# open-forest-observatory/geograypher

Measured on AMD Instinct MI355X. Metric: Mpix/s rasterized (face-ID pix2face), 1.2M-face mesh @ 4000x3000, higher is better.
Workload: dtype int32 (fixed-point edge functions) / fp32 (vertex transform, depth); 1 GPU; BASELINE config 2: 1201250-face heightfield (V=602176), 50 pinhole views/GPU @ 4000x3000, f=3000 px, 120 m AGL lawn-mower grid, face-ID raster to int32 in HBM; faces=1201250, vertices=602176, parallelism=views sharded, mesh replicated, dp1

## Files before the change

geograypher_amd/csrc/binning.hip:

```cpp
#include "gr_internal.hpp"
#include "dev_common.hpp"

using namespace grimpl;

namespace {

struct Vtx {
  int X, Y;
  float iz;
  bool valid;
  bool front, finite;
};

__device__ __forceinline__ bool snap_vertex(float qx, float qy, float iz, const float *__restrict__ cam, int gl_order, int h, int w,
                                            int &X, int &Y) {
  if (!gl_order) {
    const float fx = cam[12] * qx;
    const float fy = cam[12] * qy;
    const float sx = cam[13] + fx * iz;
    const float sy = cam[14] + fy * iz;
    X = (int)floorf(sx * 256.0f + 0.5f);
    Y = (int)floorf(sy * 256.0f + 0.5f);
    return (fabsf(sx) < 16384.0f) && (fabsf(sy) < 16384.0f);
  }
// ... 1 lines not shown
  const float px = two_f / (float)w, py = -(two_f / (float)h);
  const float hw = 0.5f * (float)w, hh = 0.5f * (float)h;
  const float xc = px * qx, yc = py * qy;
  const float xn = xc * iz, yn = yc * iz;
  const float xw = __builtin_fmaf(xn, hw, hw), yw = __builtin_fmaf(yn, hh, hh);
  const float fx = (xw - 0.5f) * 256.0f, fy = (yw - 0.5f) * 256.0f;
  X = (int)rintf(fx) + 128;
  Y = 256 * h - 128 - (int)rintf(fy);
  return (fabsf(xw) < 16384.0f) && (fabsf(yw) < 16384.0f);
}

__device__ __forceinline__ Vtx project_vertex(const float *__restrict__ p, const float *__restrict__ cam, int gl_order, int h, int w) {
  Vtx v;
  const float dx = p[0] - cam[9];
  const float dy = p[1] - cam[10];
  const float dz = p[2] - cam[11];
  float m0, m1, m2;
  m0 = cam[0] * dx; m1 = cam[3] * dy; m2 = cam[6] * dz;
  const float qx = (m0 + m1) + m2;
  m0 = cam[1] * dx; m1 = cam[4] * dy; m2 = cam[7] * dz;
  const float qy = (m0 + m1) + m2;
  m0 = cam[2] * dx; m1 = cam[5] * dy; m2 = cam[8] * dz;
  const float qz = (m0 + m1) + m2;
  v.valid = qz > cam[15];
  v.front = v.valid;
  v.finite = isfinite(qx) && isfinite(qy) && isfinite(qz);
  const float iz = 1.0f / qz;
  const bool inside = snap_vertex(qx, qy, iz, cam, gl_order, h, w, v.X, v.Y);
  v.valid = v.valid && inside;
  v.iz = iz;
  return v;
}

__device__ __forceinline__ void wave_group(int t, int lane, int &leader, int &rank, int &size) {
  leader = lane; rank = 0; size = 0;
  unsigned long long rem = __ballot(t >= 0);
  while (rem) {
    const int l = __ffsll((long long)rem) - 1;
    const int tl = __builtin_amdgcn_readlane(t, l);
    const unsigned long long m = __ballot(t == tl);
    if (t == tl) {
      leader = l;
      rank = __popcll(m & ((1ull << lane) - 1ull));
      size = __popcll(m);
    }
    rem &= ~m;
  }
}

__device__ __forceinline__ void wave_group_weighted(int t, int w, int lane, int &leader, int &rank, int &size) {
  leader = lane; rank = 0; size = 0;
  unsigned long long rem = __ballot(t >= 0);
  const unsigned long long b0 = __ballot(((w - 1) & 1) != 0), b1 = __ballot(((w - 1) & 2) != 0);
  const unsigned long long low = (1ull << lane) - 1ull;
  while (rem) {
    const int l = __ffsll((long long)rem) - 1;
    const int tl = __builtin_amdgcn_readlane(t, l);
    const unsigned long long m = __ballot(t == tl);
    if (t == tl) {
      leader = l;
      rank = __popcll(m & low) + __popcll(m & low & b0) + 2 * __popcll(m & low & b1);
      size = __popcll(m) + __popcll(m & b0) + 2 * __popcll(m & b1);
    }
    rem &= ~m;
  }
}

__device__ __forceinline__ void wave_group_capped(int t, int lane, int &leader, int &rank, int &size, int max_groups) {
  leader = lane; rank = 0; size = 1;
  unsigned long long rem = __ballot(t >= 0);
  for (int g = 0; rem && g < max_groups; ++g) {
    const int l = __ffsll((long long)rem) - 1;
    const int tl = __builtin_amdgcn_readlane(t, l);
    const unsigned long long m = __ballot(t == tl);
    if (t == tl) {
      leader = l;
      rank = __popcll(m & ((1ull << lane) - 1ull));
      size = __popcll(m);
    }
    rem &= ~m;
  }
}

__global__ __launch_bounds__(256) void k_cull_blocks(const float *__restrict__ cams, BinArgs a, int nblk) {
  const int slot = blockIdx.y;
  const int b = blockIdx.x * 256 + threadIdx.x;
  const float *cam = cams + (int64_t)slot * GR_CAM_FLOATS;
  uint32_t *ctrl = a.ctrl + slot * a.ctrl_stride;
  bool keep = false;
  if (b < nblk) {
    const float4 sp = a.blk[b];
    const float dx = sp.x - cam[9], dy = sp.y - cam[10], dz = sp.z - cam[11];
    const float qx = cam[0] * dx + cam[3] * dy + cam[6] * dz;
    const float qy = cam[1] * dx + cam[4] * dy + cam[7] * dz;
    const float qz = cam[2] * dx + cam[5] * dy + cam[8] * dz;
    const float fe = fabsf(cam[12]), r = sp.w * 1.001f;
    const float mxl = cam[13] + 2.0f, mxr = (float)a.w - cam[13] + 2.0f;
    const float myt = cam[14] + 2.0f, myb = (float)a.h - cam[14] + 2.0f;
    bool out = (qz + r < cam[15]);
    out = out || (cam[12] * qx + mxl * qz < -r * (fe + fabsf(mxl)));
    out = out || (-cam[12] * qx + mxr * qz < -r * (fe + fabsf(mxr)));
    out = out || (cam[12] * qy + myt * qz < -r * (fe + fabsf(myt)));
    out = out || (-cam[12] * qy + myb * qz < -r * (fe + fabsf(myb)));
    keep = !out;
  }
  const unsigned long long m = __ballot(keep);
  if (m != 0ull) {
    const int lane = threadIdx.x & 63;
    const int leader = __ffsll((long long)m) - 1;
    uint32_t base = 0;
    if (lane == leader) base = atomicAdd(&ctrl[3], (uint32_t)__popcll(m));
    base = __shfl(base, leader);
    if (keep) a.work[(int64_t)slot * a.work_stride + base + __popcll(m & ((1ull << lane) - 1ull))] = (uint32_t)b;
  }
}

struct FaceForm {
  int Xf, Yf, dxf, dyf, tf, rf;
  int Xm, Ym, dxm, dym, tm, rm;
  int Xl, Yl, dxl, dyl, tl, rl;
  int X0, Y0;
  int w3, w4, w5;
  int ywf;
  bool fast;
  int jmin, jmax, imin, imax;
  int iz0, A, B, nface;
};

__device__ __forceinline__ FaceForm face_form(const int4 p0, const int4 p1, const int4 p2, int TW, int TH);
__device__ __forceinline__ bool tile_entry(const FaceForm &ff, int px0, int py0, int TW, int TH, int4 &e0, int4 &e1, int4 &e2,
                                           int &rows);
__device__ __forceinline__ bool compile_entry(const BinArgs &a, uint32_t *__restrict__ ctrl, int4 *__restrict__ comp,
                                              uint8_t *__restrict__ nr8, int64_t idx, const int4 p0, const int4 p1,
                                              const int4 p2, int px0, int py0, int TW, int TH);
__device__ __forceinline__ bool build_entry(const int4 p0, const int4 p1, const int4 p2, int px0, int py0, int TW, int TH,
                                            int4 &e0, int4 &e1, int4 &e2, int &rows);
__device__ __forceinline__ void store_entry(const BinArgs &a, uint32_t *__restrict__ ctrl, int4 *__restrict__ comp,
                                            uint8_t *__restrict__ nr8, int64_t idx, const int4 e0, const int4 e1, const int4 e2,
                                            int rows);
__device__ __forceinline__ void shifted_entry(const int4 b0, const int4 b1, const int4 b2, int boxx, int boxy, int px0, int py0, int dX,
                                              int dY, int TW, int TH, int4 &e0, int4 &e1, int4 &e2, int &rows);
#define GR_FAST_EXT 24000
__device__ __forceinline__ int pack16(int lo, int hi) { return (lo & 0xFFFF) | (hi << 16); }

__device__ __forceinline__ bool face_setup_tail(const BinArgs &a, int face_id, Vtx v0, Vtx v1, Vtx v2, int4 &r0, int4 &r1,
                                                int4 &r2, int &tx0, int &tx1, int &ty0, int &ty1, bool &clip_me) {
  clip_me = !(v0.valid && v1.valid && v2.valid) && (v0.front || v1.front || v2.front) && v0.finite && v1.finite && v2.finite;
  if (!(v0.valid && v1.valid && v2.valid)) return false;
  long long area2 = (long long)(v1.X - v0.X) * (long long)(v2.Y - v0.Y) - (long long)(v2.X - v0.X) * (long long)(v1.Y - v0.Y);
  if (area2 == 0) return false;
  if (area2 < 0) {
    Vtx s = v1; v1 = v2; v2 = s;
    area2 = -area2;
  }
  const int Xmin = imin3(v0.X, v1.X, v2.X), Xmax = imax3(v0.X, v1.X, v2.X);
  const int Ymin = imin3(v0.Y, v1.Y, v2.Y), Ymax = imax3(v0.Y, v1.Y, v2.Y);
  int jmin = (Xmin - 128 + 255) >> 8, jmax = (Xmax - 128) >> 8;
  int imin = (Ymin - 128 + 255) >> 8, imax = (Ymax - 128) >> 8;
  jmin = max(jmin, 0); imin = max(imin, 0);
  jmax = min(jmax, a.w - 1); imax = min(imax, a.h - 1);
  if (jmin > jmax || imin > imax) return false;
  const double d1 = (double)v1.iz - (double)v0.iz;
  const double d2 = (double)v2.iz - (double)v0.iz;
  const double a2 = (double)area2;
  double n1, n2;
  n1 = d1 * (double)(v2.Y - v0.Y); n2 = d2 * (double)(v1.Y - v0.Y);
  const float A = (float)((n1 - n2) / a2);
// ... 669 lines not shown
      const float dx = p[0] - cam[9], dy = p[1] - cam[10], dz = p[2] - cam[11];
      float m0, m1, m2;
      m0 = cam[0] * dx; m1 = cam[3] * dy; m2 = cam[6] * dz;
      px[0][k][tid] = (double)((m0 + m1) + m2);
      m0 = cam[1] * dx; m1 = cam[4] * dy; m2 = cam[7] * dz;
      py[0][k][tid] = (double)((m0 + m1) + m2);
      m0 = cam[2] * dx; m1 = cam[5] * dy; m2 = cam[8] * dz;
      pz[0][k][tid] = (double)((m0 + m1) + m2);
    }
    int n = 3, cur = 0;
    bool bad = false;
#pragma unroll
    for (int pl = 0; pl < 5; ++pl) {
      const double pa = pl == 1 ? -(double)fe : pl == 2 ? (double)fe : 0.0;
      const double pb = pl == 3 ? -(double)fe : pl == 4 ? (double)fe : 0.0;
      const double pc = pl == 0 ? 1.0 : pl == 1 ? G - (double)cxp : pl == 2 ? G + (double)cxp : pl == 3 ? G - (double)cyp
                                                                                                        : G + (double)cyp;
      const double pd = pl == 0 ? -(double)nearp : 0.0;
      const double plane[4] = {pa, pb, pc, pd};
      if (n == 0 || bad) break;
      int m = 0;
      for (int e = 0; e < n; ++e) {
        const int e1 = (e + 1) % n;
        const P3 S = {px[cur][e][tid], py[cur][e][tid], pz[cur][e][tid]};
        const P3 E = {px[cur][e1][tid], py[cur][e1][tid], pz[cur][e1][tid]};
        const double dS = clip_plane(plane, S), dE = clip_plane(plane, E);
        const bool inS = dS >= 0.0, inE = dE >= 0.0;
        P3 o0 = E, o1 = E;
        int cnt = 0;
        if (inS && inE) { cnt = 1; }
        else if (inS && !inE) { o0 = clip_cross(S, dS, E, dE); cnt = 1; }
        else if (!inS && inE) { o0 = clip_cross(E, dE, S, dS); cnt = 2; }
        if (cnt >= 1) { if (m < 8) { px[cur ^ 1][m][tid] = o0.x; py[cur ^ 1][m][tid] = o0.y; pz[cur ^ 1][m][tid] = o0.z; } ++m; }
        if (cnt == 2) { if (m < 8) { px[cur ^ 1][m][tid] = o1.x; py[cur ^ 1][m][tid] = o1.y; pz[cur ^ 1][m][tid] = o1.z; } ++m; }
      }
      if (m > 8) bad = true;
      n = m;
      cur ^= 1;
    }
    if (bad || n < 3) continue;
    for (int e = 0; e < n; ++e) {
      const float qx = (float)px[cur][e][tid], qy = (float)py[cur][e][tid], qz = (float)pz[cur][e][tid];
      if (!(qz > 0.0f)) { bad = true; break; }
      const float iz = 1.0f / qz;
      int Xs, Ys;
      if (!snap_vertex(qx, qy, iz, cam, a.gl_order, a.h, a.w, Xs, Ys)) { bad = true; break; }
      sX[e][tid] = Xs;
      sY[e][tid] = Ys;
      sZ[e][tid] = iz;
    }
    if (bad) continue;
    const int face = a.orig[f];
    Vtx v0;
    v0.X = sX[0][tid]; v0.Y = sY[0][tid]; v0.iz = sZ[0][tid]; v0.valid = v0.front = v0.finite = true;
    for (int k = 1; k + 1 < n; ++k) {
      Vtx v1 = v0, v2 = v0;
      v1.X = sX[k][tid]; v1.Y = sY[k][tid]; v1.iz = sZ[k][tid];
      v2.X = sX[k + 1][tid]; v2.Y = sY[k + 1][tid]; v2.iz = sZ[k + 1][tid];
      emit_triangle<DIRECT>(a, slot, ctrl, v0, v1, v2, face);
    }
  }
}

__global__ __launch_bounds__(256) void k_bin_init(uint4 *__restrict__ ctrl16, int64_t n16, uint32_t *__restrict__ touched, int64_t nt,
                                                  unsigned long long *__restrict__ stats) {
  const int64_t i0 = (int64_t)blockIdx.x * 256 + threadIdx.x, step = (int64_t)gridDim.x * 256;
  for (int64_t i = i0; i < n16; i += step) ctrl16[i] = make_uint4(0u, 0u, 0u, 0u);
  for (int64_t i = i0; i < nt; i += step) touched[i] = 0u;
  if (stats && i0 < 11) stats[i0] = i0 == 4 ? ~0ull : 0ull;
}

__global__ __launch_bounds__(256) void k_sum_visits(const uint32_t *__restrict__ visits, int64_t n, unsigned long long *__restrict__ out) {
  unsigned long long sum = 0;
  for (int64_t i = (int64_t)blockIdx.x * 256 + threadIdx.x; i < n; i += (int64_t)gridDim.x * 256) sum += visits[i];
  for (int o = 32; o > 0; o >>= 1) sum += __shfl_xor(sum, o);
  if ((threadIdx.x & 63) == 0 && sum) atomicAdd(out, sum);
}

}

namespace grimpl {

int bin_batch(gr_ctx *c, const float *cams, int nb, int h, int w, int slot0, int group, hipStream_t s) {
  BinArgs a = make_args(c, h, w, slot0);
  a.group = group;
  {
    const int64_t n16 = c->ctrl_stride * nb / 4;
    const int64_t nt = a.touched ? (int64_t)nb * a.tw : 0;
    const unsigned blocks = (unsigned)std::max<int64_t>(1, std::min<int64_t>(ceil_div(std::max(n16, nt), 256), 2048));
    unsigned long long *const st = c->stats_pending ? c->stats : nullptr;
    GR_LAUNCH_EV((hipEvent_t) nullptr, chain_begin(c), k_bin_init, dim3(blocks), dim3(256), 0, s, reinterpret_cast<uint4 *>(a.ctrl), n16, a.touched, nt, st);
    c->stats_pending = false;
  }
  if (a.dbg & 512) {
    GR_HIP(c, hipMemsetAsync(a.comp, 0xFF, sizeof(int4) * GR_ENT_Q * (size_t)c->ent_cap * nb, s));
    GR_HIP(c, hipMemsetAsync(a.nrow8, 0xFF, (size_t)c->ent_cap * nb, s));
  }
  {
    const int nblk = (int)ceil_div(c->F, GR_BLOCK);
    hipLaunchKernelGGL(k_cull_blocks, dim3((unsigned)ceil_div(nblk, 256), nb), dim3(256), 0, s,
                       cams, a, nblk);
    const int gmax = std::min((nblk + 3) / 4, 1024);
    const dim3 gsetup((unsigned)std::max(1, std::min(gmax, std::max(nblk / 128, 4096 / std::max(nb, 1)))), nb);
    if (a.cap_tile > 0) {
      if (a.micro) hipLaunchKernelGGL((k_setup_cull<true, true>), gsetup, dim3(256), 0, s, cams, a);
      else hipLaunchKernelGGL((k_setup_cull<true, false>), gsetup, dim3(256), 0, s, cams, a);
      GR_LAUNCH_EV((hipEvent_t) nullptr, chain_stop(c, ST_SETUP), k_clip_faces<true>, dim3(8, nb), dim3(64), 0, s, cams, a);
    } else {
      hipLaunchKernelGGL((k_setup_cull<false, false>), gsetup, dim3(256), 0, s, cams, a);
      GR_LAUNCH_EV((hipEvent_t) nullptr, chain_stop(c, ST_SETUP), k_clip_faces<false>, dim3(8, nb), dim3(64), 0, s, cams, a);
    }
  }
  c->last_direct = a.cap_tile > 0;
  if (a.cap_tile > 0) {
    if (c->defer_stats) {
      c->stats_deferred = true; c->deferred_args = a; c->deferred_nb = nb;
    } else {
      GR_LAUNCH_EV((hipEvent_t) nullptr, chain_stop(c, ST_SCAN), k_bin_stats, dim3(nb), dim3(1024), 0, s, a);
    }
  } else {
    GR_LAUNCH_EV((hipEvent_t) nullptr, chain_stop(c, ST_SCAN), k_scan_tiles, dim3(nb), dim3(1024), 0, s, a);
    {
      const unsigned g = (unsigned)std::min<int64_t>(ceil_div(c->F, 256), 1024);
      GR_LAUNCH_EV((hipEvent_t) nullptr, chain_stop(c, ST_FILL), k_fill_compile, dim3(g, nb), dim3(256), 0, s, a);
    }
  }
  GR_HIP(c, hipGetLastError());
  return GR_OK;
}

int sum_visits(gr_ctx *c, hipStream_t s) {
  if (!c->visits_pending) return GR_OK;
  c->visits_pending = false;
  hipLaunchKernelGGL(k_sum_visits, dim3(64), dim3(256), 0, s, c->visits, ceil_div(c->F, 64), c->stats + 7);
  GR_HIP(c, hipGetLastError());
  return GR_OK;
}

int bin_stats_deferred(gr_ctx *c, hipStream_t s) {
  if (!c->stats_deferred) return GR_OK;
  c->stats_deferred = false;
  hipLaunchKernelGGL(k_bin_stats, dim3(c->deferred_nb), dim3(1024), 0, s, c->deferred_args);
  GR_HIP(c, hipGetLastError());
  return GR_OK;
}

}
```

geograypher_amd/csrc/geograster.hip:

```cpp

#include <unistd.h>

#include <mutex>
#include <new>

#include "gr_internal.hpp"

using namespace grimpl;

namespace {

std::mutex g_learned_mu;
gr_ctx::Learned g_learned[64];
int g_n_learned = 0;
char g_learned_path[1024] = {0};

#define GR_LEARNED_EXACT (-1)
#define GR_LEARNED_MAX_CAP 65536

inline int merge_cap(int a, int b) { return (a == GR_LEARNED_EXACT || b == GR_LEARNED_EXACT) ? GR_LEARNED_EXACT : std::max(a, b); }

void put_global_locked(const gr_ctx::Learned &v);

bool parse_learned_line(const char *line, gr_ctx::Learned &v) {
// ... 27 lines not shown

void put_global_locked(const gr_ctx::Learned &v) {
  int j = 0;
  for (; j < std::min(g_n_learned, 64); ++j)
    if (g_learned[j].mesh == v.mesh && g_learned[j].T == v.T) break;
  if (j == std::min(g_n_learned, 64)) {
    j = g_n_learned % 64; g_n_learned += 1;
    g_learned[j] = v;
    return;
  }
  g_learned[j].cap = merge_cap(g_learned[j].cap, v.cap);
  g_learned[j].full = g_learned[j].full || v.full;
  g_learned[j].micro = g_learned[j].micro || v.micro;
}

void lookup_learned(const gr_ctx *c, int T, int &cap, bool &full, bool *micro = nullptr) {
  cap = 0; full = false;
  if (micro) *micro = false;
  for (int i = 0; i < std::min(c->n_learned, 8); ++i)
    if (c->learned[i].mesh == c->mesh_sig && c->learned[i].T == T) {
      cap = c->learned[i].cap; full = c->learned[i].full;
      if (micro) *micro = c->learned[i].micro;
      return;
    }
  if (c->share_learned) {
    std::lock_guard<std::mutex> lk(g_learned_mu);
    for (int i = 0; i < std::min(g_n_learned, 64); ++i)
      if (g_learned[i].mesh == c->mesh_sig && g_learned[i].T == T) {
        cap = g_learned[i].cap; full = g_learned[i].full;
        if (micro) *micro = g_learned[i].micro;
        return;
      }
  }
}

void resolve_binning(gr_ctx *c, int T) {
  int cap = 0; bool full = false, micro = false;
  c->cur_cap = 0; c->cur_ent40 = false; c->cur_micro = false; c->cur_look = false; c->cur_count_micro = false;
  if (c->opt_direct_cap <= 0 || !c->direct_ok) return;
  lookup_learned(c, T, cap, full, &micro);
  if (cap == GR_LEARNED_EXACT) return;
  c->cur_look = cap == 0 && !(c->opt_var & 16384);
  c->cur_cap = std::max(cap, c->opt_direct_cap);
  c->cur_ent40 = !(c->cur_cap & 63) && !(c->opt_var & 128) && !full;
  c->cur_micro = c->cur_ent40 && !(c->opt_var & 4096) && (micro || (c->opt_var & 8192));
  c->cur_count_micro = c->cur_ent40 && !c->cur_micro && !(c->opt_var & 4096) && (c->cur_look || (c->opt_var & 16384));
}

void learn(gr_ctx *c, int T, int cap, bool full, bool micro = false) {
  int old_cap; bool old_full, old_micro;
  lookup_learned(c, T, old_cap, old_full, &old_micro);
  const gr_ctx::Learned v = {c->mesh_sig, T, merge_cap(cap, old_cap), full || old_full, micro || old_micro};
  int i = 0;
  for (; i < std::min(c->n_learned, 8); ++i)
    if (c->learned[i].mesh == c->mesh_sig && c->learned[i].T == T) break;
  if (i == std::min(c->n_learned, 8)) { i = c->n_learned % 8; c->n_learned += 1; }
  c->learned[i] = v;
  if (!c->share_learned) return;
  std::lock_guard<std::mutex> lk(g_learned_mu);
  put_global_locked(v);
  save_learned_locked();
}

void learn_slots(gr_ctx *c, int T, int64_t max_tile, bool full, bool micro) {
  const int64_t need = (max_tile + max_tile / 8 + 16 + 63) / 64 * 64;
  const int64_t bytes_one_view = need * (16 * GR_ENT_Q) * (int64_t)T;
  if (need <= GR_LEARNED_MAX_CAP && bytes_one_view <= (c->opt_budget_mb << 20)) learn(c, T, (int)need, full, micro);
  else learn(c, T, GR_LEARNED_EXACT, full, micro);
}

int ensure_bins(gr_ctx *c, int n_slots, int T) {
  const int64_t F = c->F > 0 ? c->F : 1;
  const int dcap = c->cur_cap;
  const bool direct = dcap > 0;
  int64_t cap = c->ent_cap_request > 0 ? c->ent_cap_request : (F / 2 + 65536);
  if (direct) cap = std::max<int64_t>(cap, (int64_t)T * dcap);
  int clg = -1;
  if (direct && !(c->opt_var & 131072)) {
    if (T <= 1024) { clg = 0; while ((1 << clg) < T + 3) ++clg; }
  }
  const int Tcap = clg < 0 ? ((T + 3) & ~3) : (32 << clg);
  const int64_t ctrl_stride = ((GR_CTRL_HDR + (direct ? 2 : 4) * (int64_t)Tcap) + 63) / 64 * 64;
  const int64_t work_stride = ceil_div(F, GR_BLOCK) + 4;
  int rc = grow(c, c->ctrl, c->ctrl_have, ctrl_stride * n_slots, "bin control");
  if (!rc) rc = grow(c, c->comp, c->comp_have, GR_ENT_Q * cap * n_slots, "entry list");
  if (!rc) rc = grow(c, c->nrow8, c->nrow_have, cap * n_slots + 64, "entry row counts");
  if (!rc) rc = grow(c, c->work, c->work_have, work_stride * n_slots, "work list");
  if (!rc) rc = grow(c, c->clip, c->clip_have, F * n_slots, "clip list");
  const int64_t RF = std::max<int64_t>(F, c->rec_cap_request);
  if (!rc && !direct) rc = grow(c, c->rec, c->rec_have, 4 * RF * n_slots, "record planes");
  if (rc) return rc;
  c->slots = n_slots; c->Tcap = Tcap; c->clg = clg; c->ent_cap = cap; c->ctrl_stride = ctrl_stride; c->work_stride = work_stride;
  c->rec_F = RF; c->rec_stride = 4 * RF;
  return GR_OK;
}

int raster_views(gr_ctx *c, const float *cams, int n_views, int h, int w, int32_t *ids, float *depth,
                 const uint8_t *labels, int C, uint32_t *votes, uint32_t *counts, int flags, hipStream_t s, int again = 0) {
  int rc = check_common(c, n_views, h, w);
  if (rc) return rc;
  c->rebinned = again;
  if (again == 0) c->causes = 0;
  if (!c->verts) return fail(c, GR_ENOMESH, "gr_mesh_upload has not been called");
  if (!cams) return fail(c, GR_EINVAL, "null cams");
  if (n_views == 0) return GR_OK;
  GR_HIP(c, hipSetDevice(c->device));
  int B = n_views < c->opt_batch ? n_views : c->opt_batch;
  const int thl = c->opt_thl;
  const int T = ((w + GR_TILE - 1) >> GR_TILE_LOG2) * ((h + (1 << thl) - 1) >> thl);
  resolve_binning(c, T);
  {
    const int64_t per_slot = (int64_t)T * c->cur_cap * (16 * GR_ENT_Q);
    if (per_slot > 0) B = (int)std::max<int64_t>(1, std::min<int64_t>(B, (c->opt_budget_mb << 20) / per_slot));
  }
  rc = ensure_bins(c, B, T);
  if (rc) return rc;
  c->last_T = T; c->last_B = B;
  const int64_t P = (int64_t)h * w, F = c->F;
  const bool overlap = labels && n_views > B && !(c->opt_var & 4);
  const int tw = (int)ceil_div(ceil_div(F, 64), 4);
  const bool use_touched = labels != nullptr;
  if (labels) {
    rc = ensure_winner(c, sizeof(uint32_t) * (size_t)F * B * (overlap ? 2 : 1), s);
    if (rc) return rc;
    if (use_touched) {
      rc = grow(c, c->touched, c->touched_have, (int64_t)2 * B * tw, "winner group maps");
      if (!rc) rc = grow(c, c->visits, c->visits_have, ceil_div(F, 64) + 4, "visit counters");
      if (rc) return rc;
      if (again == 0) GR_HIP(c, hipMemsetAsync(c->visits, 0, sizeof(uint32_t) * (size_t)(ceil_div(F, 64) + 4), s));
      c->visits_pending = true;
    }
    if (overlap && !c->side) {
      GR_HIP(c, hipStreamCreateWithFlags(&c->side, hipStreamNonBlocking));
      for (int i = 0; i < 2; ++i) {
        GR_HIP(c, hipEventCreateWithFlags(&c->ev_raster[i], hipEventDisableTiming));
        GR_HIP(c, hipEventCreateWithFlags(&c->ev_vote[i], hipEventDisableTiming));
      }
    }
  }
  c->last_stream = s;
  note_stream(c, s);
  c->stats_pending = true;
  c->stats_deferred = false;
  if (!labels) c->visits_pending = false;
  c->defer_stats = !labels && n_views <= B && !(c->cur_look && again < 2);
  c->last_n_views = n_views;
  int g = 0;
  for (int v0 = 0; v0 < n_views; v0 += B, ++g) {
    const int nb = (n_views - v0) < B ? (n_views - v0) : B;
    const int buf = overlap ? (g & 1) : 0;
    uint32_t *tch = use_touched ? c->touched + (int64_t)buf * B * tw : nullptr;
    if (tch) {
      if (overlap && g >= 2) GR_HIP(c, hipStreamWaitEvent(s, c->ev_vote[buf], 0));
    }
    c->cur_touched = tch; c->cur_tw = tw;
    rc = bin_batch(c, cams + (int64_t)v0 * GR_CAM_FLOATS, nb, h, w, 0, v0 / B, s);
    c->cur_touched = nullptr;
    if (rc) return rc;
    if (c->cur_look && g == 0 && again < 2) {
      unsigned long long st[11] = {0, 0, 0, 0, 0, 0, 0, 0, 0, 0, 0};
      GR_HIP(c, hipMemcpyAsync(st, c->stats, sizeof(st), hipMemcpyDeviceToHost, s));
      GR_HIP(c, hipStreamSynchronize(s));
      c->causes |= (int)(st[10] & 7u);
      const bool grow = st[3] && (int64_t)st[2] > c->cur_cap, miss = st[3] && st[5] != 0;
      const bool micro = !c->cur_micro && !(c->opt_var & (128 | 4096)) && !miss && st[0] > 0 && 5 * st[8] > 2 * st[0];
      if (grow) learn_slots(c, T, (int64_t)st[2], miss, micro);
      else learn(c, T, c->cur_cap, miss, micro);
      if (grow || miss || micro) return raster_views(c, cams, n_views, h, w, ids, depth, labels, C, votes, counts, flags, s, again + 1);
    }
    uint32_t *win = labels ? (uint32_t *)c->winner + (int64_t)buf * F * B : nullptr;
    RasterOut out;
    out.ids = ids ? ids + v0 * P : nullptr;
    out.depth = depth ? depth + v0 * P : nullptr;
    out.winner = win;
    out.touched = reinterpret_cast<uint8_t *>(tch);
    out.tb = 4 * (int64_t)tw;
    out.F = F;
    out.compat = (flags & GR_FLAG_NEG1_IS_LAST_FACE) ? 1 : 0;
    if (overlap && g >= 2) GR_HIP(c, hipStreamWaitEvent(s, c->ev_vote[buf], 0));
    rc = tile_batch(c, nb, h, w, 0, out, s);
    if (rc) return rc;
    if (labels) {
      hipStream_t vs = s;
      if (overlap) {
        GR_HIP(c, hipEventRecord(c->ev_raster[buf], s));
        GR_HIP(c, hipStreamWaitEvent(c->side, c->ev_raster[buf], 0));
        vs = c->side;
      }
      launch_vote_labels(c, vs, win, labels + v0 * P, nb, F, P, C, votes, counts, v0 / B, (const uint32_t *)tch, tw, flags);
      GR_HIP(c, hipGetLastError());
      if (overlap) GR_HIP(c, hipEventRecord(c->ev_vote[buf], c->side));
    }
  }
  if (overlap) {
    GR_HIP(c, hipStreamWaitEvent(s, c->ev_vote[(g - 1) & 1], 0));
    if (g >= 2) GR_HIP(c, hipStreamWaitEvent(s, c->ev_vote[g & 1], 0));
  }
  return GR_OK;
}

}

extern "C" {

int gr_version(void) { return GR_VERSION; }

int gr_ctx_create(int device, gr_ctx **out) {
  if (!out) return GR_EINVAL;
  *out = nullptr;
  int n = 0;
  if (hipGetDeviceCount(&n) != hipSuccess || n <= 0 || device < 0 || device >= n) return GR_ENODEVICE;
  if (hipSetDevice(device) != hipSuccess) return GR_ENODEVICE;
  gr_ctx *c = new (std::nothrow) gr_ctx();
  if (!c) return GR_ENOMEM;
  c->device = device;
  if (hipMalloc(&c->stats, sizeof(unsigned long long) * 16) != hipSuccess ||
      hipMalloc(&c->flag, sizeof(int) * 8) != hipSuccess) {
    delete c;
    return GR_ENOMEM;
  }
  (void)hipMemset(c->stats, 0, sizeof(unsigned long long) * 16);
  (void)hipDeviceSynchronize();
#ifdef GR_STAMPS
  if (hipMalloc(&c->stamps, sizeof(unsigned long long) * 32 * 1024) == hipSuccess) (void)hipMemset(c->stamps, 0, sizeof(unsigned long long) * 32 * 1024);
#endif
  *out = c;
  return GR_OK;
}

int gr_ctx_destroy(gr_ctx *c) {
  if (!c) return GR_OK;
  (void)hipSetDevice(c->device);
  (void)hipDeviceSynchronize();
  for (auto &sp : c->spans) { if (sp.own_a) (void)hipEventDestroy(sp.a); (void)hipEventDestroy(sp.b); }
  for (auto e : c->pool) (void)hipEventDestroy(e);
  if (c->ctrl) (void)hipFree(c->ctrl);
  if (c->rec) (void)hipFree(c->rec);
  if (c->comp) (void)hipFree(c->comp);
  if (c->nrow8) (void)hipFree(c->nrow8);
  if (c->work) (void)hipFree(c->work);
  if (c->clip) (void)hipFree(c->clip);
  if (c->winner) (void)hipFree(c->winner);
  for (int i = 0; i < 2; ++i) {
    if (c->ev_raster[i]) (void)hipEventDestroy(c->ev_raster[i]);
    if (c->ev_vote[i]) (void)hipEventDestroy(c->ev_vote[i]);
  }
  if (c->side) (void)hipStreamDestroy(c->side);
  if (c->sort_tmp) (void)hipFree(c->sort_tmp);
  if (c->resize_tmp) (void)hipFree(c->resize_tmp);
  if (c->blk) (void)hipFree(c->blk);
// ... 38 lines not shown
    case GR_OPT_DIRECT_CAP:
      if (value < 0 || value > 65536) return fail(c, GR_EINVAL, "slots per tile must be in [0, 65536]");
      c->opt_direct_cap = value; c->direct_ok = true; c->n_learned = 0; c->share_learned = false; return GR_OK;
    case GR_OPT_SHARE_LEARNED:
      c->share_learned = value != 0; return GR_OK;
    case GR_OPT_VERTEX_ORDER:
      if (value != 0 && value != 1) return fail(c, GR_EINVAL, "vertex order must be 0 (rule R1) or 1 (OpenGL's order of operations)");
      c->opt_gl_order = value; return GR_OK;
    case GR_OPT_DIRECT_BUDGET_MB:
      if (value < 1) return fail(c, GR_EINVAL, "entry-memory budget must be at least 1 MiB");
      c->opt_budget_mb = value; return GR_OK;
    default: return fail(c, GR_EINVAL, "unknown option %d", key);
  }
}

int gr_learned_cache_file(const char *path_h) {
  std::lock_guard<std::mutex> lk(g_learned_mu);
  if (!path_h || !path_h[0]) { g_learned_path[0] = 0; return GR_OK; }
  if (strlen(path_h) >= sizeof(g_learned_path)) return GR_EINVAL;
  snprintf(g_learned_path, sizeof(g_learned_path), "%s", path_h);
  FILE *f = fopen(path_h, "r");
  if (!f) return GR_OK;
  char line[256];
  gr_ctx::Learned v;
  while (fgets(line, sizeof(line), f))
    if (parse_learned_line(line, v)) put_global_locked(v);
  fclose(f);
  return GR_OK;
}

int gr_learned_cache_clear(void) {
  std::lock_guard<std::mutex> lk(g_learned_mu);
  g_n_learned = 0;
  memset(g_learned, 0, sizeof(g_learned));
  return GR_OK;
}

#ifdef GR_STAMPS
int gr_debug_read_stamps(gr_ctx *c, unsigned long long *out16_h) {
  if (!c || !out16_h || !c->stamps) return GR_EINVAL;
  GR_HIP(c, hipDeviceSynchronize());
  std::vector<unsigned long long> all(16 * 1024);
  GR_HIP(c, hipMemcpy(all.data(), c->stamps, sizeof(unsigned long long) * all.size(), hipMemcpyDeviceToHost));
  GR_HIP(c, hipMemset(c->stamps, 0, sizeof(unsigned long long) * all.size()));
  for (int k = 0; k < 16; ++k) out16_h[k] = 0;
  for (size_t i = 0; i < all.size(); ++i) out16_h[i & 15] += all[i];
  return GR_OK;
}
#endif

#ifdef GR_STAMPS
int gr_debug_read_setup_stamps(gr_ctx *c, unsigned long long *out16_h) {
  if (!c || !out16_h || !c->stamps) return GR_EINVAL;
  GR_HIP(c, hipDeviceSynchronize());
  std::vector<unsigned long long> all(16 * 1024);
  GR_HIP(c, hipMemcpy(all.data(), c->stamps + 16 * 1024, sizeof(unsigned long long) * all.size(), hipMemcpyDeviceToHost));
  GR_HIP(c, hipMemset(c->stamps + 16 * 1024, 0, sizeof(unsigned long long) * all.size()));
  for (int k = 0; k < 16; ++k) out16_h[k] = 0;
  for (size_t i = 0; i < all.size(); ++i) out16_h[i & 15] += all[i];
  return GR_OK;
}
#endif

int gr_get_stage_times(gr_ctx *c, gr_stage_times *o) {
  if (!c || !o) return GR_EINVAL;
  float acc[ST_N] = {0};
  for (auto &sp : c->spans) {
    GR_HIP(c, hipEventSynchronize(sp.b));
    float ms = 0.f;
    GR_HIP(c, hipEventElapsedTime(&ms, sp.a, sp.b));
    acc[sp.stage] += ms;
  }
  o->setup_ms = acc[ST_SETUP]; o->scan_ms = acc[ST_SCAN]; o->fill_ms = acc[ST_FILL]; o->raster_ms = acc[ST_RASTER];
  o->project_ms = acc[ST_PROJECT]; o->vote_ms = acc[ST_VOTE]; o->gather_ms = acc[ST_GATHER];
  o->raster_launches = c->prof_raster_launches; o->views = c->prof_views;
  release_spans(c);
  c->prof_views = 0; c->prof_raster_launches = 0;
  return GR_OK;
}

int gr_raster_face_ids(gr_ctx *c, const float *cams, int n_views, int h, int w, int32_t *ids, float *depth,
                       void *stream) {
  if (c && !ids && !depth) return fail(c, GR_EINVAL, "null outputs");
  return raster_views(c, cams, n_views, h, w, ids, depth, nullptr, 0, nullptr, nullptr, 0, (hipStream_t)stream);
}

int gr_raster_status(gr_ctx *c, gr_raster_stats *o) {
  if (!c || !o) return GR_EINVAL;
  unsigned long long st[11] = {0, 0, 0, 0, 0, 0, 0, 0, 0, 0, 0};
  {
    int rc = bin_stats_deferred(c, c->last_stream);
    if (!rc) rc = sum_visits(c, c->last_stream);
    if (rc) return rc;
  }
  GR_HIP(c, hipMemcpyAsync(st, c->stats, sizeof(st), hipMemcpyDeviceToHost, c->last_stream));
  GR_HIP(c, hipStreamSynchronize(c->last_stream));
  o->records = (int64_t)st[0]; o->entries = (int64_t)st[1]; o->max_entries = (int64_t)st[2];
  o->entry_cap = c->ent_cap; o->overflow = (int32_t)st[3];
  o->blocks = (int64_t)st[6]; o->chunk_visits = (int64_t)st[7];
  o->rebinned_groups = c->rebinned;
  c->causes |= (int)(st[10] & 7u);
  o->views_done = st[3] ? (int32_t)std::min<unsigned long long>(st[4] * (unsigned long long)std::max(c->last_B, 1),
                                                                (unsigned long long)c->last_n_views)
                        : c->last_n_views;
  if (st[3] && c->last_direct) {
    const int used = c->cur_cap;
    const bool grow = (int64_t)st[2] > used;
    if (st[5] != 0) learn(c, c->last_T, 0, true);
    if (grow) {
      learn_slots(c, c->last_T, (int64_t)st[2], false, false);
      return fail(c, GR_EOVERFLOW, "single-pass binning overflow: a tile received %llu entries (slots per tile %d); "
                  "retry the call", st[2], used);
    }
    return fail(c, GR_EOVERFLOW, "single-pass binning: a face does not fit the 40-byte entry form; retry the call "
                "(48-byte entries from now on)");
  }
  if (!st[3] && c->last_direct && c->cur_ent40 && !c->cur_micro && !(c->opt_var & 4096) && st[0] > 0 && 5 * st[8] > 2 * st[0])
    learn(c, c->last_T, 0, false, true);
  if (st[3] && (int64_t)st[9] > c->rec_F) {
    c->rec_cap_request = (int64_t)st[9] + (int64_t)st[9] / 8 + 64;
    if ((int64_t)st[2] > c->ent_cap) c->ent_cap_request = (int64_t)st[2] + (int64_t)st[2] / 8 + 65536;
    return fail(c, GR_EOVERFLOW, "record list overflow: a view needs %llu records (a clipped face becomes several triangles), "
                "capacity %lld; retry the call", st[9], (long long)c->rec_F);
  }
  if (st[3]) {
    c->ent_cap_request = (int64_t)st[2] + (int64_t)st[2] / 8 + 65536;
    return fail(c, GR_EOVERFLOW, "bin list overflow: a view needs %llu entries, capacity %lld; retry the call",
                st[2], (long long)c->ent_cap);
  }
  return GR_OK;
}

int gr_raster_overflow_causes(const gr_ctx *c) { return c ? c->causes : 0; }

int gr_raster_project_labels_u8(gr_ctx *c, const float *cams, const uint8_t *labels, int n_views, int h, int w, int C,
                                uint32_t *votes, uint32_t *counts, int32_t *ids_or_null, int flags, void *stream) {
  if (!c) return GR_EINVAL;
  if (!labels || !votes || !counts || C <= 0 || C > 255) return fail(c, GR_EINVAL, "bad fused project args C=%d", C);
  return raster_views(c, cams, n_views, h, w, ids_or_null, nullptr, labels, C, votes, counts, flags, (hipStream_t)stream);
}

}
```

geograypher_amd/csrc/gr_internal.hpp:

```cpp
#pragma once
#include <hip/hip_runtime.h>
#include <hip/hip_ext.h>

#include <algorithm>
#include <cmath>
#include <cstdarg>
#include <cstdint>
#include <cstdio>
#include <cstring>
#include <vector>

#include "geograster.h"

#define GR_TILE 64
#define GR_TILE_LOG2 6
#define GR_MAX_BATCH 64
#define GR_ENT_Q 3
#define GR_CTRL_HDR 8
#define GR_MAX_DIM 16384
#define GR_BLOCK 64
#define GR_BLOCK_VERTS 192
namespace grimpl {

struct BinArgs {
// ... 2 lines not shown
  const float *soup;
  const float *bvert;
  const uint32_t *bidx;
  const int32_t *orig;
  const float4 *blk;
  uint32_t *touched;
  int tw;
  uint32_t *work;
  uint32_t *clip;
  int64_t work_stride;
  int4 *comp;
  uint8_t *nrow8;
  unsigned long long *stats;
  int group;
  int64_t ctrl_stride;
  int64_t rec_stride;
  int64_t ent_cap;
  int64_t F;
  int T, TX, TY, Tcap;
  int clg;
  int h, w;
  int twl, thl;
  int cap_tile;
  int ent40;
  int count_micro;
  int micro;
  int var;
  int gl_order;
#ifdef GR_STAMPS
  unsigned long long *stamps;
#endif
  int dbg;
};

__device__ __forceinline__ int64_t cidx(const BinArgs &a, int t) {
  return a.clg < 0 ? (int64_t)t : (int64_t)((((uint32_t)t & ((1u << a.clg) - 1u)) << 5) | ((uint32_t)t >> a.clg));
}

struct RasterOut {
  int32_t *ids;
  float *depth;
  uint32_t *winner;
  uint8_t *touched;
  int64_t tb;
  int64_t F;
  int compat;
};

}

struct gr_ctx {
  int device = 0;
  const float *verts = nullptr;
  const int32_t *faces = nullptr;
  int64_t V = 0, F = 0;
  uint32_t *ctrl = nullptr;
  int4 *rec = nullptr;
  int4 *comp = nullptr;
  uint8_t *nrow8 = nullptr;
  int64_t nrow_have = 0;
  uint32_t *work = nullptr;
  int64_t work_stride = 0;
  uint32_t *clip = nullptr;
  int64_t clip_have = 0;
  float4 *blk = nullptr;
  uint32_t *touched = nullptr;
  uint32_t *visits = nullptr;
  int64_t visits_have = 0;
  bool visits_pending = false;
  int64_t touched_have = 0;
  uint32_t *cur_touched = nullptr;
  int cur_tw = 0;
  int64_t blk_cap = 0;
  float *soup = nullptr;
  float *bvert = nullptr;
  uint32_t *bidx = nullptr;
  int32_t *orig = nullptr;
  int64_t soup_cap = 0;
  unsigned long long *stats = nullptr;
  int *flag = nullptr;
  int64_t ctrl_stride = 0, rec_stride = 0, ent_cap = 0, ent_cap_request = 0;
  int64_t ctrl_have = 0, comp_have = 0, work_have = 0, rec_have = 0;
  int Tcap = 0, slots = 0, clg = -1;
  int64_t rec_F = 0;
  int64_t rec_cap_request = 0;
  int opt_thl = 5;
  int opt_batch = GR_MAX_BATCH;
  int opt_dbg = 0;
  int opt_var = 0;
  int opt_gl_order = 0;
  int opt_lds_pad = 0;
  int opt_direct_cap = 512;
  struct Learned { uint64_t mesh; int T, cap; bool full; bool micro = false; };
  Learned learned[8] = {};
  int n_learned = 0;
  bool share_learned = true;
  uint64_t mesh_sig = 0;
  int cur_cap = 0;
  bool cur_ent40 = false;
  bool cur_micro = false;
  bool cur_count_micro = false;
  bool cur_look = false;
  int rebinned = 0;
  int causes = 0;
  bool stats_pending = false;
  bool defer_stats = false;
  bool stats_deferred = false;
  grimpl::BinArgs deferred_args;
  int deferred_nb = 0;
  int64_t opt_budget_mb = 24 << 10;
  int last_T = 0, last_B = 0;
  int last_n_views = 0;
  bool direct_ok = true;
  bool last_direct = false;
  void *winner = nullptr;
  size_t winner_bytes = 0;
  hipStream_t side = nullptr;
  hipEvent_t ev_raster[2] = {nullptr, nullptr}, ev_vote[2] = {nullptr, nullptr};
  void *sort_tmp = nullptr;
  size_t sort_bytes = 0;
#ifdef GR_STAMPS
  unsigned long long *stamps = nullptr;
#endif
  double *resize_tmp = nullptr;
  int64_t resize_have = 0;
  hipStream_t last_stream = nullptr;
  std::vector<hipStream_t> used_streams;
  bool profiling = false;
  struct Span { hipEvent_t a, b; int stage; bool own_a = true; };
  hipEvent_t chain_ev = nullptr;
  bool chain_first = false;
  std::vector<Span> spans;
  std::vector<hipEvent_t> pool;
  int prof_views = 0, prof_raster_launches = 0;
  char err[512] = {0};
};

namespace grimpl {

inline int fail(gr_ctx *c, int code, const char *fmt, ...) {
  if (c) {
    va_list ap;
    va_start(ap, fmt);
    vsnprintf(c->err, sizeof(c->err), fmt, ap);
    va_end(ap);
  }
  return code;
}

#define GR_HIP(ctx, call)                                                                          \
  do {                                                                                             \
    hipError_t e_ = (call);                                                                        \
    if (e_ != hipSuccess) return fail(ctx, GR_EHIP, "%s: %s", #call, hipGetErrorString(e_));       \
  } while (0)

enum { ST_SETUP = 0, ST_SCAN, ST_FILL, ST_RASTER, ST_PROJECT, ST_VOTE, ST_GATHER, ST_N };

inline hipEvent_t take_event(gr_ctx *c) {
  hipEvent_t e;
  if (!c->pool.empty()) { e = c->pool.back(); c->pool.pop_back(); return e; }
  if (hipEventCreate(&e) != hipSuccess) return nullptr;
  return e;
}

struct Timed {
  gr_ctx *c; hipStream_t s; int stage; hipEvent_t a = nullptr, b = nullptr;
  Timed(gr_ctx *c_, hipStream_t s_, int st) : c(c_), s(s_), stage(st) {
    if (c->profiling && st >= 0) { a = take_event(c); b = take_event(c); if (a) (void)hipEventRecord(a, s); }
  }
  ~Timed() {
    if (c->profiling && a && b) { (void)hipEventRecord(b, s); gr_ctx::Span sp; sp.a = a; sp.b = b; sp.stage = stage; c->spans.push_back(sp); }
  }
};

inline hipEvent_t chain_begin(gr_ctx *c) {
  if (c->chain_ev && c->chain_first) c->pool.push_back(c->chain_ev);
  c->chain_ev = c->profiling ? take_event(c) : nullptr;
  c->chain_first = true;
  return c->chain_ev;
}
inline hipEvent_t chain_stop(gr_ctx *c, int stage) {
  if (!c->profiling || !c->chain_ev) return nullptr;
  hipEvent_t e = take_event(c);
  if (!e) return nullptr;
  gr_ctx::Span sp; sp.a = c->chain_ev; sp.b = e; sp.stage = stage; sp.own_a = c->chain_first;
  c->spans.push_back(sp);
  c->chain_first = false;
  c->chain_ev = e;
  return e;
}
inline void release_spans(gr_ctx *c) {
  if (c->chain_ev && c->chain_first) c->pool.push_back(c->chain_ev);
  c->chain_ev = nullptr; c->chain_first = false;
  for (auto &sp : c->spans) { if (sp.own_a) c->pool.push_back(sp.a); c->pool.push_back(sp.b); }
  c->spans.clear();
}
#define GR_LAUNCH_EV(EVA, EVB, KERNEL, GRID, BLOCK, SHMEM, STREAM, ...)                                        \
  do {                                                                                                         \
    const hipEvent_t eva_ = (EVA), evb_ = (EVB);    \
    if (eva_ || evb_) hipExtLaunchKernelGGL(KERNEL, GRID, BLOCK, SHMEM, STREAM, eva_, evb_, 0, __VA_ARGS__);   \
    else hipLaunchKernelGGL(KERNEL, GRID, BLOCK, SHMEM, STREAM, __VA_ARGS__);                                  \
  } while (0)

inline int64_t ceil_div(int64_t a, int64_t b) { return (a + b - 1) / b; }

inline void quiesce(gr_ctx *c) {
  for (hipStream_t st : c->used_streams) (void)hipStreamSynchronize(st);
  c->used_streams.clear();
  if (c->side) (void)hipStreamSynchronize(c->side);
}

inline void note_stream(gr_ctx *c, hipStream_t s) {
  for (hipStream_t st : c->used_streams)
    if (st == s) return;
  c->used_streams.push_back(s);
}

template <typename T>
int grow(gr_ctx *c, T *&ptr, int64_t &have, int64_t want, const char *what) {
  if (ptr && have >= want) return GR_OK;
  if (ptr) quiesce(c);
  if (ptr) (void)hipFree(ptr);
  ptr = nullptr; have = 0;
  if (hipMalloc(&ptr, sizeof(T) * (size_t)want) != hipSuccess)
    return fail(c, GR_ENOMEM, "%s scratch allocation failed (%lld bytes)", what, (long long)(sizeof(T) * (size_t)want));
  have = want;
  return GR_OK;
}

inline int ensure_winner(gr_ctx *c, size_t bytes, hipStream_t s) {
  if (c->winner && c->winner_bytes >= bytes) return GR_OK;
  if (c->winner) quiesce(c);
  if (c->winner) (void)hipFree(c->winner);
  c->winner = nullptr; c->winner_bytes = 0;
  if (hipMalloc(&c->winner, bytes) != hipSuccess) return fail(c, GR_ENOMEM, "winner scratch allocation failed");
  if (hipMemsetAsync(c->winner, 0, bytes, s) != hipSuccess) return fail(c, GR_EHIP, "winner memset failed");
  c->winner_bytes = bytes;
  return GR_OK;
}

inline BinArgs make_args(gr_ctx *c, int h, int w, int slot0) {
  BinArgs a;
  a.ctrl_stride = c->ctrl_stride; a.rec_stride = c->rec_stride; a.ent_cap = c->ent_cap; a.F = c->F;
  a.work_stride = c->work_stride;
  a.ctrl = c->ctrl + slot0 * a.ctrl_stride; a.rec = c->rec + slot0 * a.rec_stride;
  a.comp = c->comp + slot0 * a.ent_cap * GR_ENT_Q; a.work = c->work + slot0 * a.work_stride;
  a.nrow8 = c->nrow8 + slot0 * a.ent_cap;
  a.stats = c->stats; a.blk = c->blk; a.soup = c->soup; a.orig = c->orig; a.bvert = c->bvert; a.bidx = c->bidx;
  a.touched = c->cur_touched; a.tw = c->cur_tw;
  a.clip = c->clip + slot0 * c->F;
  a.twl = GR_TILE_LOG2; a.thl = c->opt_thl;
  a.TX = (w + (1 << a.twl) - 1) >> a.twl; a.TY = (h + (1 << a.thl) - 1) >> a.thl; a.T = a.TX * a.TY; a.Tcap = c->Tcap; a.clg = c->clg;
  a.h = h; a.w = w; a.dbg = c->opt_dbg; a.var = c->opt_var; a.gl_order = c->opt_gl_order;
  a.cap_tile = c->cur_cap;
  a.ent40 = c->cur_ent40 ? 1 : 0;
  a.micro = c->cur_micro ? 1 : 0;
  a.count_micro = c->cur_count_micro ? 1 : 0;
  a.group = 0;
#ifdef GR_STAMPS
  a.stamps = c->stamps;
#endif
  return a;
}

inline int check_common(gr_ctx *c, int n_views, int h, int w) {
  if (!c) return GR_EINVAL;
  if (n_views < 0 || h <= 0 || w <= 0 || h > GR_MAX_DIM || w > GR_MAX_DIM)
    return fail(c, GR_EINVAL, "bad shape n_views=%d h=%d w=%d (limit %d)", n_views, h, w, GR_MAX_DIM);
  return GR_OK;
}

int bin_batch(gr_ctx *c, const float *cams, int nb, int h, int w, int slot0, int group, hipStream_t s);
int tile_batch(gr_ctx *c, int nb, int h, int w, int slot0, RasterOut out, hipStream_t s);
int bin_stats_deferred(gr_ctx *c, hipStream_t s);
int sum_visits(gr_ctx *c, hipStream_t s);
int project_labels(gr_ctx *c, const int32_t *ids, const uint8_t *labels, int n_views, int h, int w, int C, uint32_t *votes,
                   uint32_t *counts, int flags, hipStream_t s);
void launch_vote_labels(gr_ctx *c, hipStream_t vs, uint32_t *win, const uint8_t *labels, int nb, int64_t F, int64_t P, int C,
                        uint32_t *votes, uint32_t *counts, int group, const uint32_t *touched, int tw, int flags);

}
```

Baseline: 697,200 Mpix/s.

## Double-buffer bin control and zero next half inside cull kernel to skip init launch

```diff
diff --git a/geograypher_amd/csrc/binning.hip b/geograypher_amd/csrc/binning.hip
--- a/geograypher_amd/csrc/binning.hip
+++ b/geograypher_amd/csrc/binning.hip
@@ -107,7 +107,15 @@
   }
 }
 
-__global__ __launch_bounds__(256) void k_cull_blocks(const float *__restrict__ cams, BinArgs a, int nblk) {
+__global__ __launch_bounds__(256) void k_cull_blocks(const float *__restrict__ cams, BinArgs a, int nblk, uint4 *__restrict__ zero16,
+                                                     int64_t n16, uint32_t *__restrict__ touched, int64_t nt,
+                                                     unsigned long long *__restrict__ stats) {
+  {
+    const int64_t i0 = ((int64_t)blockIdx.y * gridDim.x + blockIdx.x) * 256 + threadIdx.x, step = (int64_t)gridDim.x * gridDim.y * 256;
+    for (int64_t i = i0; i < n16; i += step) zero16[i] = make_uint4(0u, 0u, 0u, 0u);
+    for (int64_t i = i0; i < nt; i += step) touched[i] = 0u;
+    if (stats && i0 < 11) stats[i0] = i0 == 4 ? ~0ull : 0ull;
+  }
   const int slot = blockIdx.y;
   const int b = blockIdx.x * 256 + threadIdx.x;
   const float *cam = cams + (int64_t)slot * GR_CAM_FLOATS;
@@ -943,15 +951,20 @@
 namespace grimpl {
 
 int bin_batch(gr_ctx *c, const float *cams, int nb, int h, int w, int slot0, int group, hipStream_t s) {
+  const bool alternate = !(c->opt_var & 262144);
+  const bool clean = alternate && c->clean_half >= 0 && c->clean_stride == c->ctrl_stride && c->clean_tcap == c->Tcap &&
+                     c->clean_slots == c->slots && c->clean_clg == c->clg;
+  c->ctrl_half = clean ? c->clean_half : 0;
+  c->clean_half = -1;
   BinArgs a = make_args(c, h, w, slot0);
   a.group = group;
-  {
+  const int64_t nt = a.touched ? (int64_t)nb * a.tw : 0;
+  unsigned long long *const st = c->stats_pending ? c->stats : nullptr;
+  c->stats_pending = false;
+  if (!clean) {
     const int64_t n16 = c->ctrl_stride * nb / 4;
-    const int64_t nt = a.touched ? (int64_t)nb * a.tw : 0;
     const unsigned blocks = (unsigned)std::max<int64_t>(1, std::min<int64_t>(ceil_div(std::max(n16, nt), 256), 2048));
-    unsigned long long *const st = c->stats_pending ? c->stats : nullptr;
     GR_LAUNCH_EV((hipEvent_t) nullptr, chain_begin(c), k_bin_init, dim3(blocks), dim3(256), 0, s, reinterpret_cast<uint4 *>(a.ctrl), n16, a.touched, nt, st);
-    c->stats_pending = false;
   }
   if (a.dbg & 512) {
     GR_HIP(c, hipMemsetAsync(a.comp, 0xFF, sizeof(int4) * GR_ENT_Q * (size_t)c->ent_cap * nb, s));
@@ -959,17 +972,25 @@
   }
   {
     const int nblk = (int)ceil_div(c->F, GR_BLOCK);
-    hipLaunchKernelGGL(k_cull_blocks, dim3((unsigned)ceil_div(nblk, 256), nb), dim3(256), 0, s,
-                       cams, a, nblk);
+    uint4 *const zero16 = reinterpret_cast<uint4 *>(c->ctrl + (int64_t)(c->ctrl_half ^ 1) * c->slots * c->ctrl_stride);
+    const int64_t n16 = alternate ? c->ctrl_stride * c->slots / 4 : 0;
+    GR_LAUNCH_EV(clean ? chain_begin(c) : (hipEvent_t) nullptr, (hipEvent_t) nullptr, k_cull_blocks, dim3((unsigned)ceil_div(nblk, 256), nb),
+                 dim3(256), 0, s, cams, a, nblk, zero16, n16, clean ? a.touched : nullptr, clean ? nt : 0,
+                 clean ? st : (unsigned long long *)nullptr);
+    if (alternate) {
+      c->clean_half = c->ctrl_half ^ 1;
+      c->clean_stride = c->ctrl_stride; c->clean_tcap = c->Tcap; c->clean_slots = c->slots; c->clean_clg = c->clg;
+    }
     const int gmax = std::min((nblk + 3) / 4, 1024);
     const dim3 gsetup((unsigned)std::max(1, std::min(gmax, std::max(nblk / 128, 4096 / std::max(nb, 1)))), nb);
+    const dim3 gclip(8, nb);
     if (a.cap_tile > 0) {
       if (a.micro) hipLaunchKernelGGL((k_setup_cull<true, true>), gsetup, dim3(256), 0, s, cams, a);
       else hipLaunchKernelGGL((k_setup_cull<true, false>), gsetup, dim3(256), 0, s, cams, a);
-      GR_LAUNCH_EV((hipEvent_t) nullptr, chain_stop(c, ST_SETUP), k_clip_faces<true>, dim3(8, nb), dim3(64), 0, s, cams, a);
+      GR_LAUNCH_EV((hipEvent_t) nullptr, chain_stop(c, ST_SETUP), k_clip_faces<true>, gclip, dim3(64), 0, s, cams, a);
     } else {
       hipLaunchKernelGGL((k_setup_cull<false, false>), gsetup, dim3(256), 0, s, cams, a);
-      GR_LAUNCH_EV((hipEvent_t) nullptr, chain_stop(c, ST_SETUP), k_clip_faces<false>, dim3(8, nb), dim3(64), 0, s, cams, a);
+      GR_LAUNCH_EV((hipEvent_t) nullptr, chain_stop(c, ST_SETUP), k_clip_faces<false>, gclip, dim3(64), 0, s, cams, a);
     }
   }
   c->last_direct = a.cap_tile > 0;
diff --git a/geograypher_amd/csrc/geograster.hip b/geograypher_amd/csrc/geograster.hip
--- a/geograypher_amd/csrc/geograster.hip
+++ b/geograypher_amd/csrc/geograster.hip
@@ -133,7 +133,10 @@
   const int Tcap = clg < 0 ? ((T + 3) & ~3) : (32 << clg);
   const int64_t ctrl_stride = ((GR_CTRL_HDR + (direct ? 2 : 4) * (int64_t)Tcap) + 63) / 64 * 64;
   const int64_t work_stride = ceil_div(F, GR_BLOCK) + 4;
-  int rc = grow(c, c->ctrl, c->ctrl_have, ctrl_stride * n_slots, "bin control");
+  const uint32_t *const ctrl_was = c->ctrl;
+  const int64_t ctrl_had = c->ctrl_have;
+  int rc = grow(c, c->ctrl, c->ctrl_have, 2 * ctrl_stride * n_slots, "bin control");
+  if (c->ctrl != ctrl_was || c->ctrl_have != ctrl_had) c->clean_half = -1;
   if (!rc) rc = grow(c, c->comp, c->comp_have, GR_ENT_Q * cap * n_slots, "entry list");
   if (!rc) rc = grow(c, c->nrow8, c->nrow_have, cap * n_slots + 64, "entry row counts");
   if (!rc) rc = grow(c, c->work, c->work_have, work_stride * n_slots, "work list");
@@ -217,6 +220,7 @@
       const bool micro = !c->cur_micro && !(c->opt_var & (128 | 4096)) && !miss && st[0] > 0 && 5 * st[8] > 2 * st[0];
       if (grow) learn_slots(c, T, (int64_t)st[2], miss, micro);
       else learn(c, T, c->cur_cap, miss, micro);
+      if (grow || miss || micro) c->clean_half = -1;
       if (grow || miss || micro) return raster_views(c, cams, n_views, h, w, ids, depth, labels, C, votes, counts, flags, s, again + 1);
     }
     uint32_t *win = labels ? (uint32_t *)c->winner + (int64_t)buf * F * B : nullptr;
@@ -421,7 +425,9 @@
 int gr_raster_face_ids(gr_ctx *c, const float *cams, int n_views, int h, int w, int32_t *ids, float *depth,
                        void *stream) {
   if (c && !ids && !depth) return fail(c, GR_EINVAL, "null outputs");
-  return raster_views(c, cams, n_views, h, w, ids, depth, nullptr, 0, nullptr, nullptr, 0, (hipStream_t)stream);
+  const int rc = raster_views(c, cams, n_views, h, w, ids, depth, nullptr, 0, nullptr, nullptr, 0, (hipStream_t)stream);
+  if (rc && c) c->clean_half = -1;
+  return rc;
 }
 
 int gr_raster_status(gr_ctx *c, gr_raster_stats *o) {
@@ -439,6 +445,7 @@
   o->blocks = (int64_t)st[6]; o->chunk_visits = (int64_t)st[7];
   o->rebinned_groups = c->rebinned;
   c->causes |= (int)(st[10] & 7u);
+  if (st[3]) c->clean_half = -1;
   o->views_done = st[3] ? (int32_t)std::min<unsigned long long>(st[4] * (unsigned long long)std::max(c->last_B, 1),
                                                                 (unsigned long long)c->last_n_views)
                         : c->last_n_views;
@@ -476,7 +483,9 @@
                                 uint32_t *votes, uint32_t *counts, int32_t *ids_or_null, int flags, void *stream) {
   if (!c) return GR_EINVAL;
   if (!labels || !votes || !counts || C <= 0 || C > 255) return fail(c, GR_EINVAL, "bad fused project args C=%d", C);
-  return raster_views(c, cams, n_views, h, w, ids_or_null, nullptr, labels, C, votes, counts, flags, (hipStream_t)stream);
-}
-
-}
+  const int rc = raster_views(c, cams, n_views, h, w, ids_or_null, nullptr, labels, C, votes, counts, flags, (hipStream_t)stream);
+  if (rc) c->clean_half = -1;
+  return rc;
+}
+
+}
diff --git a/geograypher_amd/csrc/gr_internal.hpp b/geograypher_amd/csrc/gr_internal.hpp
--- a/geograypher_amd/csrc/gr_internal.hpp
+++ b/geograypher_amd/csrc/gr_internal.hpp
@@ -108,6 +108,9 @@
   int64_t ctrl_stride = 0, rec_stride = 0, ent_cap = 0, ent_cap_request = 0;
   int64_t ctrl_have = 0, comp_have = 0, work_have = 0, rec_have = 0;
   int Tcap = 0, slots = 0, clg = -1;
+  int ctrl_half = 0, clean_half = -1;
+  int64_t clean_stride = 0;
+  int clean_tcap = 0, clean_slots = 0, clean_clg = -1;
   int64_t rec_F = 0;
   int64_t rec_cap_request = 0;
   int opt_thl = 5;
@@ -269,7 +272,7 @@
   BinArgs a;
   a.ctrl_stride = c->ctrl_stride; a.rec_stride = c->rec_stride; a.ent_cap = c->ent_cap; a.F = c->F;
   a.work_stride = c->work_stride;
-  a.ctrl = c->ctrl + slot0 * a.ctrl_stride; a.rec = c->rec + slot0 * a.rec_stride;
+  a.ctrl = c->ctrl + ((int64_t)c->ctrl_half * c->slots + slot0) * a.ctrl_stride; a.rec = c->rec + slot0 * a.rec_stride;
   a.comp = c->comp + slot0 * a.ent_cap * GR_ENT_Q; a.work = c->work + slot0 * a.work_stride;
   a.nrow8 = c->nrow8 + slot0 * a.ent_cap;
   a.stats = c->stats; a.blk = c->blk; a.soup = c->soup; a.orig = c->orig; a.bvert = c->bvert; a.bidx = c->bidx;
```

New measurement: 697,200 Mpix/s. Within noise of the previous version (-0.0%).
